# fenghuayumo/DIVSHOT

Hardware: AMD Instinct MI355X
Metric: train views/sec (fwd+bwd raster) at 1M splats 1920x1080 (higher is better)
Workload: dtype f32; 1 GPU; C3: 1000000 splats, 1920x1080, SH degree 3, 8 views per iteration sharded over 1 GPU(s) (BASELINE config C4), 8 view(s) per GPU per step as 1 multi-view pass(es) of 8 view(s) (dvs_raster_forward_views / dvs_raster_backward_*); absgrad=True, mode=batch, stagger=False, groups=1, views_per_group=8, early_gather=False, a9_chunks=1, async_forward=True, hip_graph=False, fwd_variant=quadrant, grad_mode=0, tile_bounds=canonical, shN_layout=tiled[N/64][45][64]

## Files before the change

divshot_amd/csrc/dvs_api.cpp:

```cpp
#include <hip/hip_runtime.h>
#include <cstddef>
#include <cstdio>
#include <cstdlib>
#include <cstdint>
#include <cstring>
#include <mutex>
#include <string>
#include <vector>
#include "../../include/dvs_raster.h"
#include "dvs_kernels.h"

static thread_local std::string g_last_error;
static void set_error(const char* what, hipError_t e, const char* file, int line) {
    char buf[512];
    snprintf(buf, sizeof buf, "%s: %s (%s:%d)", what, hipGetErrorString(e), file, line);
    g_last_error = buf;
}
void dvs_set_last_error(const char* msg) { g_last_error = msg ? msg : ""; }
static int fail(int code, const char* who, const char* what) { g_last_error = std::string(who) + ": " + what; return code; }
#define HIPCHECK(expr) do { hipError_t _e = (expr); if (_e != hipSuccess) { set_error(#expr, _e, __FILE__, __LINE__); return DVS_ERR_HIP; } } while (0)
#define TRY(expr) do { int _r = (expr); if (_r != DVS_OK) return _r; } while (0)

namespace {
struct Buf {
// ... 42 lines not shown

struct FwdPass {
    hipStream_t st;
    const dvs_splats* p; const dvs_camera* cams; int V; const dvs_opts* opts;
    int n; TileGrid g;
    uint64_t T = 0, T_expected = 0;
    const uint64_t* T_dev = nullptr;
    int icur = 0;
    int ranges_encoded = 0;
    bool keys_written = true;
};

struct Arenas {
    Buf radii, splat2d, depth, flags, tiles_touched, rect, rect_sorted, key[2], ids[2];
    Buf ranges, final_T, n_contrib;
    Buf ranges_canon;
    Buf inst_tile[2], inst_splat[2];
    uint64_t inst_cap = 0;
    uint64_t inst_grow_events = 0;
    uint64_t* total_dev = nullptr;
    uint64_t* total_host = nullptr;
    uint64_t overflow_seen = 0;
    Buf tmp_keys, tmp_vals;
};
struct FrontEnd {
    Buf state, hist;
    uint32_t nbv = 0, nsb = 0;
    int rank_atomic = 0;
    DvsSeg *seg_all = nullptr, *seg_vis = nullptr, *seg_tile = nullptr;
    uint32_t *superexcl = nullptr, *totals = nullptr, *block_sums = nullptr, *kred = nullptr, *tile_ranges = nullptr;
// ... 12 lines not shown
    size_t carve_ranges(void* base, int max_views, size_t tiles) {
        Carver k{(char*)base};
        kred = k.take<uint32_t>(DVS_FE_KRED_WORDS);
        super = k.take<unsigned long long>((size_t)max_views * nsb * DVS_FE_SUPER_STRIDE);
        zero_bytes = k.off = (k.off + 255) & ~(size_t)255;
        tile_ranges = k.take<uint32_t>(tiles * 2);
        return k.off;
    }
};
struct Forward {
    dvs_fwd_state st{};
    int n_views = 1;
    bool have = false;
    uint32_t* live_splat = nullptr;
    uint32_t* live_pos = nullptr;
    bool live_lists = true;
    uint64_t* rec_masks = nullptr; uint64_t rec_cap = 0;
    struct Prep {
        bool valid = false;
        int64_t next = 0;
        int n = 0, V = 0;
        dvs_splats p{};
        dvs_opts opts{};
        dvs_camera cams[DVS_MAX_VIEWS];
    } prep;
};
struct Backward {
    Buf g_rows;
    Buf dcolor;
    int variant = DVS_BWD_TR;
    bool keep_rows = false;
// ... 26 lines not shown
    bool async_T = false;
    bool export_tiles = false;
    Arenas a;
    FrontEnd fe;
    Forward fwd;
    Backward bwd;
    Timing timing;
    Probe probe;
    ~dvs_ctx() {
        if (a.total_dev) (void)hipFree(a.total_dev);
        if (a.total_host) (void)hipHostFree(a.total_host);
        for (const auto* pool : {&timing.events, &probe.ev}) for (hipEvent_t e : *pool) (void)hipEventDestroy(e);
    }
};

namespace {
enum : unsigned { DROP_FWD = 1u, DROP_ROWS = 2u, DROP_PREP = 4u, DROP_SEGS = 8u };
void invalidate(dvs_ctx* c, unsigned what) {
    if (what & DROP_FWD) c->fwd.have = false;
    if (what & DROP_ROWS) c->bwd.rows_pending = false;
    if (what & DROP_PREP) c->fwd.prep.valid = false;
    if (what & DROP_SEGS) c->fe.seg_n = -1;
}

struct StageScope {
    dvs_ctx* c; hipStream_t st; bool append; size_t last = 0;
    StageScope(dvs_ctx* c_, hipStream_t s, bool append_) : c(c_), st(s), append(append_) { c->timing.used = 0; c->timing.spans.clear(); }
    size_t mark() {
        Timing& t = c->timing;
        if (!t.on) return 0;
// ... 37 lines not shown
}
int ensure_splat_arenas(dvs_ctx* c, size_t n) {
    Arenas& a = c->a;
    const struct { Buf* buf; size_t each; } need[] = {{&a.radii, 4}, {&a.splat2d, 64}, {&a.depth, 4}, {&a.flags, 4}, {&a.tiles_touched, 4},
        {&a.rect, 16}, {&a.rect_sorted, 16}, {&a.key[0], 4}, {&a.key[1], 4}, {&a.ids[0], 4}, {&a.ids[1], 4}, {&c->bwd.g_rows, 48}};
    for (const auto& x : need) TRY(x.buf->ensure(n * x.each));
    return DVS_OK;
}
int ensure_image_arenas(dvs_ctx* c, int w, int h, int views) {
    const size_t P = (size_t)w * h * views;
    const size_t tiles = (size_t)TileGrid(w, h).tiles * views;
    TRY(c->a.ranges.ensure(c->fe.carve_ranges(nullptr, c->max_views, tiles)));
    c->fe.carve_ranges(c->a.ranges.p, c->max_views, tiles);
    TRY(c->a.ranges_canon.ensure(tiles * 8));
    TRY(c->a.final_T.ensure(P * 4));
    return c->a.n_contrib.ensure(P * 4);
}
int ensure_instance_arenas(dvs_ctx* c, uint64_t T) {
    Arenas& a = c->a;
    if (a.inst_cap && T > a.inst_cap) ++a.inst_grow_events;
    uint64_t cap = (1ull << 32) - 1;
    for (Buf* b : {&a.inst_tile[0], &a.inst_splat[0], &a.inst_tile[1], &a.inst_splat[1]}) {
        TRY(b->ensure(T * 4));
        if (b->bytes / 4 < cap) cap = b->bytes / 4;
    }
    a.inst_cap = cap;
    return c->fe.hist.ensure(dvs_fe_hist_words(a.inst_cap, c->max_views, 512) * 4);
}
}

// ... 151 lines not shown
        HIPCHECK(dvs_launch_seg_sort(st, V, a.inst_tile[0].as<uint32_t>(), a.inst_splat[0].as<uint32_t>(), a.inst_tile[1].as<uint32_t>(),
                                     a.inst_splat[1].as<uint32_t>(), fe.seg_tile, 0, tiles > 1 ? bits_for((uint32_t)(tiles - 1)) : 1,
                                     c->async_T ? (f.T_expected ? f.T_expected : a.inst_cap) : f.T, tile_part, nbtot, fe.hist.as<uint32_t>(), fe.totals,
                                     (uint32_t)tiles, &f.icur, fuse_a6 ? fe.tile_ranges : nullptr, f.keys_written ? 1 : 0, key16, fe.rank_atomic));
    }
    tm.stage("tile_sort");
    if (fuse_a6) f.ranges_encoded = n > 0 ? 1 : 0;
    else HIPCHECK(dvs_launch_tile_ranges(st, f.T, a.inst_tile[f.icur].as<uint32_t>(), fe.tile_ranges, f.T_dev, f.T_expected));
    tm.stage("tile_ranges");
    return DVS_OK;
}
static int fwd_composite_and_publish(dvs_ctx* c, const FwdPass& f, float* out_rgb, dvs_fwd_state* saved, uint64_t* num_rendered, StageScope& tm) {
    Arenas& a = c->a; Forward& fw = c->fwd;
    const int W = f.cams[0].width, H = f.cams[0].height, icur = f.icur;
    probe_event(c, f.st, 0);
    fw.live_splat = nullptr; fw.live_pos = nullptr;
    uint64_t* rec_masks = nullptr; uint64_t rec_cap = 0;
    if (fw.rec_masks && f.V == 1 && !c->async_T) {
        rec_masks = fw.rec_masks; rec_cap = fw.rec_cap;
        HIPCHECK(hipMemsetAsync(rec_masks, 0, (size_t)(f.T < rec_cap ? f.T : rec_cap) * 32, f.st));
    }
    if (fw.live_lists && c->bwd.variant == DVS_BWD_TR) { fw.live_splat = a.inst_splat[icur ^ 1].as<uint32_t>(); fw.live_pos = a.inst_tile[icur ^ 1].as<uint32_t>(); }
    uint32_t* const canon = f.ranges_encoded ? a.ranges_canon.as<uint32_t>() : nullptr;
    HIPCHECK(dvs_launch_render_fwd(f.st, W, H, f.g.tiles_x, f.g.tiles_y, f.V, c->fe.tile_ranges, a.inst_splat[icur].as<uint32_t>(),
                                   a.splat2d.as<float>(), CamVec3(f.cams, f.V, &dvs_camera::bg).v, out_rgb, a.final_T.as<float>(),
                                   a.n_contrib.as<uint32_t>(), fw.live_splat, fw.live_pos, rec_masks, rec_cap, canon));
    probe_event(c, f.st);
    tm.stage("render_fwd");

    dvs_fwd_state& s = fw.st;
    s.radii = a.radii.as<int32_t>(); s.splat2d = a.splat2d.as<float>(); s.depth = a.depth.as<float>();
    s.flags = a.flags.as<uint32_t>();
    s.tiles_touched = a.tiles_touched.as<uint32_t>();
    s.sorted_tile = f.keys_written ? a.inst_tile[icur].as<uint32_t>() : nullptr; s.sorted_splat = a.inst_splat[icur].as<uint32_t>();
    s.ranges = canon ? canon : c->fe.tile_ranges; s.final_T = a.final_T.as<float>(); s.n_contrib = a.n_contrib.as<uint32_t>();
    s.num_rendered = c->async_T ? DVS_T_UNKNOWN : f.T; s.n = f.n; s.width = W; s.height = H; s.tiles_x = f.g.tiles_x; s.tiles_y = f.g.tiles_y;
    s._pad = 0;
    fw.n_views = f.V;
    fw.have = true;
    if (saved) *saved = s;
    if (num_rendered) *num_rendered = s.num_rendered;
// ... 59 lines not shown
    }
    if (count <= 0 || first < 0 || first + count > p->n || (first % 256) != 0) {
        invalidate(c, DROP_PREP);
        return fail(DVS_ERR_INVALID, who, "bad chunk (each starts at a multiple of 256 and lies inside [0, n))");
    }
    HIPCHECK(hipSetDevice(c->device));
    if (begin) invalidate(c, DROP_FWD | DROP_ROWS | DROP_PREP);
    const int r = run_a2(c, (hipStream_t)stream, p, cams, n_views, opts, first, count, begin);
    if (r != DVS_OK) { invalidate(c, DROP_PREP); return r; }
    publish_prep(c, p, cams, n_views, opts, first + count);
    return DVS_OK;
}

int dvs_get_view_state(dvs_ctx* c, int view, dvs_fwd_state* out) {
    if (!c || !out) return fail(DVS_ERR_INVALID, "dvs_get_view_state", "null argument");
    if (!c->fwd.have || view < 0 || view >= c->fwd.n_views) return fail(DVS_ERR_STATE, "dvs_get_view_state", "no such view in the last forward");
    dvs_fwd_state s = c->fwd.st;
    const size_t on = (size_t)view * s.n, op = (size_t)view * s.width * s.height, ot = (size_t)view * s.tiles_x * s.tiles_y;
    s.radii += on; s.splat2d += on * DVS_S2D_FLOATS; s.depth += on; s.flags += on; s.tiles_touched += on;
    s.ranges += 2 * ot; s.final_T += op; s.n_contrib += op;
    *out = s;
    return DVS_OK;
}

static int bwd_composite(dvs_ctx* c, hipStream_t st, const dvs_camera* cams, const dvs_opts* opts, const float* dL_drgb, StageScope& tm) {
    const dvs_fwd_state& s = c->fwd.st;
    Backward& b = c->bwd;
    const int V = c->fwd.n_views;
    tm.begin();
    if (!b.rows_clean) HIPCHECK(hipMemsetAsync(b.g_rows.p, 0, b.g_rows.bytes, st));
    b.rows_clean = false;
    tm.stage("bwd_zero");
    const CamVec3 bgs(cams, V, &dvs_camera::bg);
    probe_event(c, st, 1);
    if (b.variant == DVS_BWD_TR)
        HIPCHECK(dvs_launch_render_bwd_tr(st, s.width, s.height, s.tiles_x, s.tiles_y, V, s.ranges, s.sorted_splat, s.splat2d, bgs.v, s.final_T,
                                          s.n_contrib, dL_drgb, b.g_rows.as<float>(), opts->absgrad, opts->grad_mode, c->fwd.live_splat, c->fwd.live_pos));
    else
        HIPCHECK(dvs_launch_render_bwd_blocks(st, s.width, s.height, s.tiles_x, s.tiles_y, V, s.ranges, s.sorted_splat, s.splat2d,
                                              bgs.v, s.final_T, s.n_contrib, dL_drgb, b.g_rows.as<float>(), opts->absgrad, opts->grad_mode));
    probe_event(c, st);
    tm.stage("render_bwd");
    b.rows_pending = true;
    b.proj_next = 0;
    return DVS_OK;
}
static int bwd_project(dvs_ctx* c, hipStream_t st, const dvs_splats* p, const dvs_camera* cams, const dvs_opts* opts,
                       const dvs_splat_grads* out, int64_t first, int64_t count, StageScope& tm) {
    const dvs_fwd_state& s = c->fwd.st;
    Backward& b = c->bwd;
    const int V = c->fwd.n_views, n = p->n;
    tm.begin();
// ... 251 lines not shown
    c->fwd.rec_masks = take_masks; c->fwd.rec_cap = take_masks ? capacity_instances : 0;
    return DVS_OK;
}

int dvs_set_backward_variant(dvs_ctx* c, int variant) {
    const char* const who = "dvs_set_backward_variant";
    if (!c || variant < DVS_BWD_BLOCKS || variant > DVS_BWD_TR) return fail(DVS_ERR_INVALID, who, "bad argument");
    if (variant == DVS_BWD_REDUCE || variant == DVS_BWD_MM)
        return fail(DVS_ERR_UNSUPPORTED, who, "the 'reduce' and 'mm' kernels are retired — this library contains 'tr' (default) and 'blocks' only");
    c->bwd.variant = variant;
    return DVS_OK;
}
int dvs_set_live_lists(dvs_ctx* c, int enable) {
    if (!c) return fail(DVS_ERR_INVALID, "dvs_set_live_lists", "null context");
    c->fwd.live_lists = enable != 0;
    return DVS_OK;
}
int dvs_set_forward_variant(dvs_ctx* c, int variant) {
    if (!c || (variant != 0 && variant != 1)) return fail(DVS_ERR_INVALID, "dvs_set_forward_variant", "bad argument");
    if (variant == 0)
        return fail(DVS_ERR_UNSUPPORTED, "dvs_set_forward_variant", "the per-block forward is retired — this library contains the quadrant forward only");
    return DVS_OK;
}

int dvs_keep_bwd_intermediates(dvs_ctx* c, int keep) { if (!c) return DVS_ERR_INVALID; c->bwd.keep_rows = keep != 0; return DVS_OK; }

int dvs_get_bwd_intermediates(dvs_ctx* c, const float** rows, int* row_floats) {
    if (!c) return DVS_ERR_INVALID;
    if (rows) *rows = c->bwd.g_rows.as<float>();
    if (row_floats) *row_floats = 12;
// ... 56 lines not shown
```

divshot_amd/csrc/dvs_kernels.h:

```cpp
#pragma once
#include <hip/hip_runtime.h>
#include <stdint.h>
#include "dvs_device.h"

hipError_t dvs_launch_preprocess_fwd(hipStream_t st, int n, const float* pos, const float* sh0, const float* shN,
                                     const float* opacity, const float* scale, const float* rot, const DvsCams& cams, int n_views,
                                     int deg, int antialias, int tiles_x, int tiles_y, int* radii , float* splat2d,
                                     float* depth, uint32_t* flags,
                                     uint32_t* tiles_touched, uint32_t* depth_key, int shn_tiled,
                                     uint32_t* rect , int rect_fmt ,
                                     uint32_t* kred ,
                                     int first, int count );
hipError_t dvs_launch_preprocess_bwd(hipStream_t st, int n, const float* pos, const float* shN, const float* opacity,
                                     const float* scale, const float* rot, const DvsCam& cam, int deg, int antialias,
                                     const int* radii, const uint32_t* flags, float* grad_rows ,
                                     float* g_pos, float* g_sh0, float* g_shN, float* g_opacity, float* g_scale,
                                     float* g_rot, float* out_absgrad2d , float* out_mean2d ,
                                     float* out_dcolor , int accumulate, int rezero_rows, int shn_tiled, int grad_mode);
hipError_t dvs_launch_preprocess_bwd_views(hipStream_t st, int n, int n_views, const float* pos, const float* shN, const float* opacity,
                                           const float* scale, const float* rot, const DvsCams& cams, int deg, int antialias,
                                           const int* radii, const uint32_t* flags, float* grad_rows, float* g_pos, float* g_opacity,
                                           float* g_scale, float* g_rot, float* out_absgrad2d, float* out_mean2d, float* out_dcolor,
                                           int accumulate, int rezero_rows, int grad_mode, int first, int count, float* g_sh0 ,
                                           float* g_shN );
// ... 64 lines not shown
hipError_t dvs_launch_seg_sort(hipStream_t st, int V, uint32_t* keys0, uint32_t* vals0, uint32_t* keys1, uint32_t* vals1, DvsSeg* seg, int bit_lo, int bits,
                               uint64_t grid_elems, uint32_t part, uint32_t nbtot, uint32_t* hist, uint32_t* totals, uint32_t key_add_per_view,
                               int* result_in, uint32_t* ranges_enc = nullptr ,
                               int write_last_keys = 1, int first_keys16 = 0 , int rank_atomic = 0);
hipError_t dvs_fe_probe_rank_atomic(hipStream_t st, uint32_t* bad_dev);
hipError_t dvs_launch_seg_binning(hipStream_t st, int n, int V, int rect_fmt, const DvsSeg* seg_vis, DvsSeg* seg_tile, const uint32_t* sorted_ids,
                                  const uint32_t* rect, uint32_t* rect_sorted, uint32_t* block_sums, unsigned long long* super, uint32_t* superexcl,
                                  uint32_t tile_part, unsigned long long* total_dev, unsigned long long capacity, int stage, int tiles_x,
                                  uint32_t* inst_tile, uint32_t* inst_splat, int key16 = 0 );

hipError_t dvs_launch_tile_ranges(hipStream_t st, uint64_t T, const uint32_t* sorted_tile, uint32_t* ranges ,
                                  const uint64_t* T_dev = nullptr, uint64_t T_expected = 0);
hipError_t dvs_launch_export_keys(hipStream_t st, uint64_t T, const uint32_t* sorted_tile, const uint32_t* sorted_splat,
                                  const float* depth, uint64_t* out_keys);

hipError_t dvs_launch_render_fwd(hipStream_t st, int W, int H, int tiles_x, int tiles_y, int n_views, const uint32_t* ranges ,
                                 const uint32_t* sorted_splat, const float* splat2d, const float* bgs, float* out_color, float* final_T,
                                 uint32_t* n_contrib, uint32_t* live_splat , uint32_t* live_pos ,
                                 uint64_t* take_masks ,
                                 uint64_t take_cap, uint32_t* ranges_out = nullptr );
enum { DVS_BWD_BLOCKS = 0 , DVS_BWD_REDUCE = 1 , DVS_BWD_MM = 2 ,
       DVS_BWD_TR = 3  };

hipError_t dvs_launch_render_bwd_tr(hipStream_t st, int W, int H, int tiles_x, int tiles_y, int n_views, const uint32_t* ranges,
                                    const uint32_t* sorted_splat, const float* splat2d, const float* bgs , const float* final_T,
                                    const uint32_t* n_contrib, const float* dL_dout, float* grad_rows, int absgrad, int grad_mode,
                                    const uint32_t* live_splat ,
                                    const uint32_t* live_pos);

hipError_t dvs_launch_render_bwd_blocks(hipStream_t st, int W, int H, int tiles_x, int tiles_y, int n_views, const uint32_t* ranges,
                                        const uint32_t* sorted_splat, const float* splat2d, const float* bgs , const float* final_T,
                                        const uint32_t* n_contrib, const float* dL_dout, float* grad_rows, int absgrad, int grad_mode);
```

divshot_amd/csrc/render.hip:

```cpp
#include "dvs_device.h"
#include "dvs_kernels.h"
#include "render_common.h"

struct __attribute__((aligned(16))) FwdLds {
    float4 a[RB];
    float4 b[RB];
    float4 c[RB];
    uint64_t qmask[RB / 64][4];
    uint32_t wlive[RB / 64];
};
__device__ __forceinline__ void lds_put(FwdLds& L, int t, float2 xy, float4 co, float3 col) {
    L.a[t] = make_float4(xy.x, xy.y, -0.72134752044448170f * co.x, -1.4426950408889634f * co.y);
    L.b[t] = make_float4(-0.72134752044448170f * co.z, co.w, col.x, col.y);
    L.c[t].x = col.z;
}

__device__ __forceinline__ bool stage_batch(FwdLds& L, const uint32_t* __restrict__ sorted_splat, uint32_t first, int cnt,
                                            const float4* __restrict__ splat2d, float tile_x0, float tile_y0, uint32_t& id_out) {
    const int t = threadIdx.x;
    uint32_t qm = 0;
    id_out = 0u;
    if (t < cnt) {
        const uint32_t id = sorted_splat[first + t];
        id_out = id;
// ... 37 lines not shown
}

__device__ __forceinline__ uint64_t uniform_u64(uint64_t v) {
    const uint32_t lo = __builtin_amdgcn_readfirstlane((uint32_t)v), hi = __builtin_amdgcn_readfirstlane((uint32_t)(v >> 32));
    return ((uint64_t)hi << 32) | lo;
}

template <bool RECORD>
__global__ void __launch_bounds__(RB)
k_render_fwd(ViewBg bg_arg , int W, int H, int tiles_x, int tiles_per_view,
             int num_tiles , const uint2* __restrict__ ranges, uint2* __restrict__ ranges_out ,
             const uint32_t* __restrict__ sorted_splat, const float4* __restrict__ splat2d,
             float* __restrict__ out_color , float* __restrict__ final_T , uint32_t* __restrict__ n_contrib,
             uint32_t* __restrict__ live_splat ,
             uint32_t* __restrict__ live_pos ,
             uint64_t* __restrict__ take_masks , uint64_t take_cap) {
    __shared__ FwdLds L;
    (void)bg_arg;
    const int tile_g = tile_of_block(blockIdx.x, num_tiles);
    if (tile_g >= num_tiles) return;
    const int view = tile_g / tiles_per_view, tile = tile_g - view * tiles_per_view;
    const float3 bgv = dvs_load_bg(view);
    const float bg0 = bgv.x, bg1 = bgv.y, bg2 = bgv.z;
    out_color += (size_t)view * 3 * W * H; final_T += (size_t)view * W * H; n_contrib += (size_t)view * W * H;
    const int tx = tile % tiles_x, ty = tile / tiles_x;
    const int wave = threadIdx.x >> 6, lane = threadIdx.x & 63;
    const int px = tx * DVS_TILE + (wave & 1) * 8 + (lane & 7);
    const int py = ty * DVS_TILE + (wave >> 1) * 8 + (lane >> 3);
    const bool inside = px < W && py < H;
    const float pxf = (float)px, pyf = (float)py;
    uint2 range = ranges[tile_g];
    if (ranges_out) {
        range.x = range.y ? ~range.x : 0u;
        if (threadIdx.x == 0) ranges_out[tile_g] = range;
    }
    const int total = (int)(range.y - range.x);
    uint64_t notdone = __builtin_amdgcn_ballot_w64(inside);
    float T = 1.0f, C0 = 0.f, C1 = 0.f, C2 = 0.f;
    uint32_t last = 0;
    uint32_t live_base = 0;

    for (int base = 0; base < total; base += RB) {
        if (__syncthreads_and(notdone == 0ull)) break;
        const int cnt = min(RB, total - base);
        uint32_t my_id;
        const bool live = stage_batch(L, sorted_splat, range.x + base, cnt, splat2d, (float)(tx * DVS_TILE), (float)(ty * DVS_TILE), my_id);
        const uint64_t lm = __ballot(live);
        const uint32_t lrank = __builtin_amdgcn_mbcnt_hi((uint32_t)(lm >> 32), __builtin_amdgcn_mbcnt_lo((uint32_t)lm, 0u));
        if (lane == 0) L.wlive[wave] = (uint32_t)__popcll(lm);
        __syncthreads();
        if (live_pos) {
            uint32_t pre = 0, tot = 0;
#pragma unroll
            for (int w = 0; w < RB / 64; ++w) { const uint32_t c = L.wlive[w]; pre += w < wave ? c : 0u; tot += c; }
            const uint32_t lp = live_base + pre + lrank;
            if ((int)threadIdx.x < cnt) live_pos[range.x + base + threadIdx.x] = lp;
            if (live) live_splat[range.x + lp] = my_id;
            live_base += tot;
        }
        if (notdone == 0ull) continue;
#pragma unroll 1
        for (int lw = 0; lw < RB / 64; ++lw) {
            uint64_t m = uniform_u64(L.qmask[lw][wave]);
            if (m == 0) continue;
            if (notdone == 0ull) break;
            typedef float fwd_v4f __attribute__((ext_vector_type(4)));
            typedef __attribute__((address_space(3))) const fwd_v4f lds_cv4f;
            uint32_t word_a = (uint32_t)(uintptr_t)&L.a[lw * 64];
            asm("" : "+v"(word_a));
            const int idx0 = base + lw * 64 + 1;
            uint64_t exec_entry;
            asm volatile("s_mov_b64 %0, exec" : "=s"(exec_entry));
// ... 25 lines not shown
                             "v_mov_b32 %[last], %[idx]\n\t"
                             "s_mov_b64 exec, %[ee]"
                             : [c0] "+v"(C0), [c1] "+v"(C1), [c2] "+v"(C2), [T] "+v"(T), [last] "+v"(last), [nd] "+s"(notdone)
                             : [p2] "v"(p2), [al] "v"(alpha), [tt] "v"(test_T), [cr] "v"(B.z), [cg] "v"(B.w), [cbl] "v"(cb), [at] "v"(aT), [idx] "s"(idx),
                               [amin] "s"(DVS_ALPHA_MIN), [tstop] "s"(DVS_T_STOP), [ee] "s"(exec_entry)
                             : "vcc", "scc");
                if (RECORD) {
                    const uint64_t took = nd_before & __builtin_amdgcn_ballot_w64(!(p2 > 0.f)) & __builtin_amdgcn_ballot_w64(!(alpha < DVS_ALPHA_MIN)) &
                                          ~__builtin_amdgcn_ballot_w64(test_T < DVS_T_STOP);
                    const uint64_t pos = (uint64_t)range.x + (uint64_t)(idx - 1u);
                    if (lane == 0 && pos < take_cap) take_masks[pos * 4 + wave] = took;
                }
            }
        }
    }
    if (inside) {
        const size_t P = (size_t)W * H, pix = (size_t)py * W + px;
        final_T[pix] = T;
        n_contrib[pix] = last;
        out_color[pix] = C0 + T * bg0;
        out_color[P + pix] = C1 + T * bg1;
        out_color[2 * P + pix] = C2 + T * bg2;
    }
}


hipError_t dvs_launch_render_fwd(hipStream_t st, int W, int H, int tiles_x, int tiles_y, int n_views, const uint32_t* ranges,
                                 const uint32_t* sorted_splat, const float* splat2d, const float* bgs, float* out_color, float* final_T,
                                 uint32_t* n_contrib, uint32_t* live_splat, uint32_t* live_pos, uint64_t* take_masks, uint64_t take_cap, uint32_t* ranges_out) {
    const int tiles_pv = tiles_x * tiles_y, num_tiles = tiles_pv * n_views;
    if (num_tiles <= 0) return hipSuccess;
    const int grid = ((num_tiles + 7) >> 3) << 3;
    if (take_masks)
        hipLaunchKernelGGL(k_render_fwd<true>, dim3(grid), dim3(RB), 0, st, make_view_bg(n_views, bgs), W, H, tiles_x, tiles_pv, num_tiles,
                           (const uint2*)ranges, (uint2*)ranges_out, sorted_splat, (const float4*)splat2d, out_color, final_T, n_contrib, live_splat, live_pos, take_masks, take_cap);
    else
        hipLaunchKernelGGL(k_render_fwd<false>, dim3(grid), dim3(RB), 0, st, make_view_bg(n_views, bgs), W, H, tiles_x, tiles_pv, num_tiles,
                           (const uint2*)ranges, (uint2*)ranges_out, sorted_splat, (const float4*)splat2d, out_color, final_T, n_contrib, live_splat, live_pos, (uint64_t*)nullptr, (uint64_t)0);
    return hipGetLastError();
}
```

divshot_amd/csrc/render_tr.hip:

```cpp
#include "dvs_device.h"
#include "dvs_kernels.h"
#include "render_common.h"

#define TR_SLOTS 4
#define TR_SS 136
#define TR_MINW 6

template <int BK>
struct __attribute__((aligned(16))) TrLds {
    float4 ea[BK + 1];
    float4 eb[BK + 1];
    float4 ec[BK + 1];
    uint2 idop[2][BK];
    uint8_t list[(BK + 1) * 16];
    uint32_t cnt[16];
    uint32_t blast[16];
};

template <int BK>
__device__ __forceinline__ uint32_t tr_load_id(const uint32_t* __restrict__ sorted_splat, uint32_t first, int cnt) {
    const int e = threadIdx.x % BK;
    return e < cnt ? sorted_splat[first + e] : 0u;
}
template <int BK>
// ... 48 lines not shown
            len = (uint32_t)__popc(up ? hi : lo);
        }
        if (hit) L.list[(rk + 1u) * 16u + (uint32_t)(b0 + i)] = (uint8_t)e;
        if (e == 0) L.cnt[b0 + i] = len;
    }
}

template <bool ABSGRAD, bool LINEAGE, int BK>
__global__ void __launch_bounds__(RB, TR_MINW)
k_render_bwd_tr(ViewBg bg_arg , int W, int H, int tiles_x, int tiles_per_view,
                int num_tiles , const uint2* __restrict__ ranges,
                const uint32_t* __restrict__ sorted_splat, const float4* __restrict__ splat2d,
                const float* __restrict__ final_T, const uint32_t* __restrict__ n_contrib, const float* __restrict__ dL_dout ,
                float* __restrict__ grow ,
                const uint32_t* __restrict__ live_splat ,
                const uint32_t* __restrict__ live_pos ) {
    __shared__ TrLds<BK> L;
    __shared__ __attribute__((aligned(16))) float s_tab[4][(BK + 1) * 12];
    __shared__ __attribute__((aligned(16))) float s_tb[4][TR_SLOTS * TR_SS];
    (void)bg_arg;
    const int tile_g = tile_of_block(blockIdx.x, num_tiles);
    if (tile_g >= num_tiles) return;
    const int view = tile_g / tiles_per_view, tile = tile_g - view * tiles_per_view;
    const float3 bgv = dvs_load_bg(view);
    final_T += (size_t)view * W * H; n_contrib += (size_t)view * W * H; dL_dout += (size_t)view * 3 * W * H;
    const int tx = tile % tiles_x, ty = tile / tiles_x;
    const int wave = threadIdx.x >> 6, lane = threadIdx.x & 63;
    const size_t P = (size_t)W * H;
    const int g1 = lane >> 4, pi = lane & 15;
    const int bx1 = 2 * (wave & 1) + (g1 & 1), by1 = 2 * (wave >> 1) + (g1 >> 1), blk1 = by1 * 4 + bx1;
    const int px = tx * DVS_TILE + 4 * bx1 + (pi & 3), py = ty * DVS_TILE + 4 * by1 + (pi >> 2);
    const bool inside = px < W && py < H;
    const size_t pix = (size_t)py * W + px;
    const float pxf = (float)px, pyf = (float)py;
    const uint2 range = ranges[tile_g];
    const int r2 = lane >> 4, s2 = (lane >> 2) & 3, g2 = lane & 3;
    const int bx2 = 2 * (wave & 1) + (g2 & 1), by2 = 2 * (wave >> 1) + (g2 >> 1);
    const int X0 = tx * DVS_TILE + 4 * bx2, Y0 = ty * DVS_TILE + 4 * by2 + r2;
    const float X0f = (float)X0, Y0f = (float)Y0;
    float d2[4][3];
    if ((W & 3) == 0) {
        const bool in2 = X0 < W && Y0 < H;
        const size_t q = (size_t)Y0 * W + X0;
#pragma unroll
        for (int c = 0; c < 3; ++c) {
            const float4 v = in2 ? *reinterpret_cast<const float4*>(dL_dout + c * P + q) : make_float4(0.f, 0.f, 0.f, 0.f);
            d2[0][c] = v.x; d2[1][c] = v.y; d2[2][c] = v.z; d2[3][c] = v.w;
        }
    } else {
#pragma unroll
        for (int x = 0; x < 4; ++x) {
            const bool in2 = X0 + x < W && Y0 < H;
            const size_t q = (size_t)Y0 * W + X0 + x;
#pragma unroll
            for (int c = 0; c < 3; ++c) d2[x][c] = in2 ? dL_dout[c * P + q] : 0.f;
        }
    }
    const int perm_r = (r2 == 1) ? 2 : (r2 == 2) ? 1 : r2;
    const int xaddr = (lane ^ 32) << 2;
    const int jaddr = (16 * g2) << 2;
    const uint32_t jshift = 8u * (uint32_t)(TR_SLOTS - 1 - s2);

    const float T_final = inside ? final_T[pix] : 0.f;
    uint32_t last = inside ? n_contrib[pix] : 0u;
    if (live_pos) {
        if (last > 0u) last = live_pos[range.x + last - 1u] + 1u;
        sorted_splat = live_splat;
    }
    float dLp0 = 0.f, dLp1 = 0.f, dLp2 = 0.f;
    if (inside) { dLp0 = dL_dout[pix]; dLp1 = dL_dout[P + pix]; dLp2 = dL_dout[2 * P + pix]; }
    const float bg_dot = (bgv.x * dLp0 + bgv.y * dLp1) + bgv.z * dLp2;

    uint32_t bmax = last;
#pragma unroll
    for (int d = 8; d >= 1; d >>= 1) bmax = max(bmax, (uint32_t)__shfl_xor((int)bmax, d, 64));
    if (pi == 0) L.blast[blk1] = bmax;
    for (int e = threadIdx.x; e < (BK + 1) * 12; e += RB) reinterpret_cast<float4*>(&s_tab[0][0])[e] = make_float4(0.f, 0.f, 0.f, 0.f);
    if (threadIdx.x < 16) L.list[threadIdx.x] = (uint8_t)BK;
    if (threadIdx.x == 0) { L.ea[BK] = make_float4(0.f, 0.f, 0.f, 0.f); L.eb[BK] = make_float4(0.f, 0.f, 0.f, 0.f); L.ec[BK] = make_float4(0.f, 0.f, 0.f, 0.f); }
    __syncthreads();
    uint32_t todo = 0;
#pragma unroll
    for (int g = 0; g < 16; ++g) todo = max(todo, L.blast[g]);
    if (todo == 0) return;

    float T = T_final;
    float D = T_final * bg_dot;
    const uint32_t tb_m0 = (uint32_t)__builtin_amdgcn_readfirstlane((int)(uint32_t)(uintptr_t)&s_tb[wave][0]);
    typedef __attribute__((address_space(3))) float lds_float;
    typedef float tr_v4f __attribute__((ext_vector_type(4)));
    typedef __attribute__((address_space(3))) const tr_v4f lds_cv4f;
    uint32_t tbr_a = (uint32_t)(uintptr_t)&s_tb[wave][TR_SS * s2 + 16 * g2 + 4 * r2];
    uint32_t tabw_a = (uint32_t)(uintptr_t)&s_tab[wave][perm_r];
    asm("" : "+v"(tbr_a), "+v"(tabw_a));
    const uint8_t* const lbase = &L.list[0];

    auto flush = [&](uint32_t jpack) {
        const uint32_t jp = (uint32_t)__builtin_amdgcn_ds_bpermute(jaddr, (int)jpack);
        const int j = (int)((jp >> jshift) & 0xffu);
// ... 36 lines not shown
        }
        const float q0 = swap16_add(h0, h1), q1 = swap16_add(h2, h3), q2 = swap16_add(h4, h5);
        uint32_t slot_a;
        asm("v_mad_u32_u24 %0, %1, 48, %2" : "=v"(slot_a) : "v"(j), "v"(tabw_a));
        lds_float* const slot = (lds_float*)slot_a;
#pragma unroll
        for (int g = 0; g < 4; ++g) {
            if (g2 == g) { slot[0] += q0; slot[4] += q1; slot[8] += q2; }
            __builtin_amdgcn_wave_barrier();
            asm volatile("" ::: "memory");
        }
    };

    const int nbatch = (int)((todo + BK - 1) / BK);
    const float tile_x0 = (float)(tx * DVS_TILE), tile_y0 = (float)(ty * DVS_TILE);
    uint32_t id_stage = tr_load_id<BK>(sorted_splat, range.x + (nbatch - 1) * BK, min(BK, (int)todo - (nbatch - 1) * BK));
    for (int b = nbatch - 1; b >= 0; --b) {
        const int base = b * BK;
        const int cnt = min(BK, (int)todo - base);
        tr_stage<BK>(L, splat2d, id_stage, cnt, base, b & 1, tile_x0, tile_y0);
        __syncthreads();
        const int len = (int)L.cnt[blk1];
        int nmax = len;
        nmax = max(nmax, __shfl_xor(nmax, 16, 64));
        nmax = max(nmax, __shfl_xor(nmax, 32, 64));
        nmax = __builtin_amdgcn_readfirstlane(nmax);
        const int lastb = (int)min(last, (uint32_t)(base + BK)) - base;
        uint32_t p = (uint32_t)len * 16u + (uint32_t)blk1;
        uint32_t jn = lbase[p];
        asm("" : "+v"(jn));
        uint32_t jpack = 0;
// ... 43 lines not shown
            const float val = (s_tab[0][e] + s_tab[1][e]) + (s_tab[2][e] + s_tab[3][e]);
            if (val != 0.f) {
                const int ent = e / 12, comp = e - 12 * ent;
                const uint2 io = L.idop[b & 1][ent];
                const float sc = (comp == 5 || (comp >= 6 && comp <= 8)) ? 1.f : __uint_as_float(io.y);
                if (comp < 11) atomicAdd(&grow[(size_t)io.x * 12 + comp], val * sc);
            }
            s_tab[0][e] = 0.f; s_tab[1][e] = 0.f; s_tab[2][e] = 0.f; s_tab[3][e] = 0.f;
        }
    }
}

hipError_t dvs_launch_render_bwd_tr(hipStream_t st, int W, int H, int tiles_x, int tiles_y, int n_views, const uint32_t* ranges,
                                    const uint32_t* sorted_splat, const float* splat2d, const float* bgs, const float* final_T,
                                    const uint32_t* n_contrib, const float* dL_dout, float* grad_rows, int absgrad, int grad_mode,
                                    const uint32_t* live_splat, const uint32_t* live_pos) {
    const int tiles_pv = tiles_x * tiles_y, num_tiles = tiles_pv * n_views;
    if (num_tiles <= 0) return hipSuccess;
    const int grid = ((num_tiles + 7) >> 3) << 3;
    const int lineage = grad_mode == 1 ? 1 : 0;
#define DVS_TR(A, LN, BKV)                                                                                                              \
    hipLaunchKernelGGL((k_render_bwd_tr<A, LN, BKV>), dim3(grid), dim3(RB), 0, st, make_view_bg(n_views, bgs), W, H, tiles_x, tiles_pv, \
                       num_tiles, (const uint2*)ranges, sorted_splat, (const float4*)splat2d, final_T, n_contrib, dL_dout, grad_rows, live_splat, live_pos)
#define DVS_TR_B(BKV)                                                                                   \
    do {                                                                                                \
        if (absgrad) { if (lineage) DVS_TR(true, true, BKV); else DVS_TR(true, false, BKV); }           \
        else { if (lineage) DVS_TR(false, true, BKV); else DVS_TR(false, false, BKV); }                 \
    } while (0)
    DVS_TR_B(64);
#undef DVS_TR_B
#undef DVS_TR
    return hipGetLastError();
}
```

include/dvs_raster.h:

```cpp
#ifndef DVS_RASTER_H
#define DVS_RASTER_H

#include <stddef.h>
#include <stdint.h>

#ifdef __cplusplus
extern "C" {
#endif

#define DVS_TILE 16
#define DVS_SH_REST 15

enum {
    DVS_OK = 0,
    DVS_ERR_INVALID = 1,
    DVS_ERR_HIP = 2,
    DVS_ERR_CAPACITY = 3,
    DVS_ERR_STATE = 4,
    DVS_ERR_UNSUPPORTED = 5
};

typedef struct dvs_splats {
    const float* pos;
    const float* sh0;
// ... 87 lines not shown

int dvs_sh_grad_combine(dvs_ctx* ctx, void* stream, int n, const float* pos, int sh_degree, int n_views, const float* campos,
                        const float* dcolor, float* g_sh0, float* g_shN, int accumulate, int shn_layout);
int dvs_shn_relayout(dvs_ctx* ctx, void* stream, int n, const float* src, float* dst, int to_tiled);

dvs_ctx* dvs_create_views(int device, size_t max_splats, int max_w, int max_h, int max_views);
int dvs_raster_forward_views(dvs_ctx* ctx, void* stream, const dvs_splats* params, const dvs_camera* cams, int n_views,
                             const dvs_opts* opts, float* out_rgb);
int dvs_raster_backward_views(dvs_ctx* ctx, void* stream, const dvs_splats* params, const dvs_camera* cams, int n_views,
                              const dvs_opts* opts, const float* dL_drgb, const dvs_splat_grads* out);

int dvs_raster_forward_views_prepare(dvs_ctx* ctx, void* stream, const dvs_splats* params, const dvs_camera* cams, int n_views,
                                     const dvs_opts* opts, int64_t first, int64_t count);
int dvs_raster_forward_cancel_prepared(dvs_ctx* ctx);
int dvs_get_view_state(dvs_ctx* ctx, int view, dvs_fwd_state* state);

#define DVS_T_UNKNOWN (~0ull)
int dvs_set_async(dvs_ctx* ctx, int enable);
int dvs_get_num_rendered(dvs_ctx* ctx, void* stream, uint64_t* num_rendered);
int dvs_get_arena_info(dvs_ctx* ctx, uint64_t* instance_capacity, uint64_t* grow_events, uint64_t* last_num_rendered, uint64_t* overflows);
int dvs_get_sort_rank_mode(dvs_ctx* ctx);
int dvs_set_export_sorted_tiles(dvs_ctx* ctx, int enable);

int dvs_debug_record_decisions(dvs_ctx* ctx, uint64_t* take_masks, uint64_t capacity_instances);
int dvs_debug_sort_depth_keys(dvs_ctx* ctx, void* stream, const uint32_t* keys, uint64_t n, uint32_t* sorted_ids, uint32_t* n_sorted, uint32_t* digit_bits);

int dvs_set_backward_variant(dvs_ctx* ctx, int variant);
int dvs_set_forward_variant(dvs_ctx* ctx, int variant);
int dvs_set_live_lists(dvs_ctx* ctx, int enable);

// ... 24 lines not shown
```

Measured before the change: 1830 views/s.

## Hand off per-pixel live count and per-tile block maxima from forward to backward

The forward render kernel now also writes a compacted per-pixel last-live index and a per-tile header holding the tile's todo count and its 16 block maxima. The backward TR kernel reads these instead of gathering live_pos through n_contrib and reducing block maxima with shuffles and LDS, and it issues the first id stage load earlier. This removes a dependent indirect load and a reduction plus sync from the backward prologue. In exchange the forward kernel gains extra LDS, shuffles, a barrier and additional global writes of a pixel-sized buffer.

```diff
diff --git a/divshot_amd/csrc/dvs_api.cpp b/divshot_amd/csrc/dvs_api.cpp
--- a/divshot_amd/csrc/dvs_api.cpp
+++ b/divshot_amd/csrc/dvs_api.cpp
@@ -80,6 +80,7 @@
 struct Arenas {
     Buf radii, splat2d, depth, flags, tiles_touched, rect, rect_sorted, key[2], ids[2];
     Buf ranges, final_T, n_contrib;
+    Buf last_live, tile_head;
     Buf ranges_canon;
     Buf inst_tile[2], inst_splat[2];
     uint64_t inst_cap = 0;
@@ -122,7 +123,10 @@
     bool have = false;
     uint32_t* live_splat = nullptr;
     uint32_t* live_pos = nullptr;
+    uint32_t* last_live = nullptr;
+    DvsTileHead* tile_head = nullptr;
     bool live_lists = true;
+    bool use_handoff = true;
     uint64_t* rec_masks = nullptr; uint64_t rec_cap = 0;
     struct Prep {
         bool valid = false;
@@ -179,6 +183,7 @@
     }
 };
 
+static_assert(sizeof(DvsTileHead) == 4 * DVS_TILE_HEAD_WORDS, "dvs_raster.h describes the tile header to the tests");
 namespace {
 enum : unsigned { DROP_FWD = 1u, DROP_ROWS = 2u, DROP_PREP = 4u, DROP_SEGS = 8u };
 void invalidate(dvs_ctx* c, unsigned what) {
@@ -246,6 +251,8 @@
     c->fe.carve_ranges(c->a.ranges.p, c->max_views, tiles);
     TRY(c->a.ranges_canon.ensure(tiles * 8));
     TRY(c->a.final_T.ensure(P * 4));
+    TRY(c->a.last_live.ensure(P * 4));
+    TRY(c->a.tile_head.ensure(tiles * sizeof(DvsTileHead)));
     return c->a.n_contrib.ensure(P * 4);
 }
 int ensure_instance_arenas(dvs_ctx* c, uint64_t T) {
@@ -427,17 +434,18 @@
     Arenas& a = c->a; Forward& fw = c->fwd;
     const int W = f.cams[0].width, H = f.cams[0].height, icur = f.icur;
     probe_event(c, f.st, 0);
-    fw.live_splat = nullptr; fw.live_pos = nullptr;
+    fw.live_splat = nullptr; fw.live_pos = nullptr; fw.last_live = nullptr; fw.tile_head = nullptr;
     uint64_t* rec_masks = nullptr; uint64_t rec_cap = 0;
     if (fw.rec_masks && f.V == 1 && !c->async_T) {
         rec_masks = fw.rec_masks; rec_cap = fw.rec_cap;
         HIPCHECK(hipMemsetAsync(rec_masks, 0, (size_t)(f.T < rec_cap ? f.T : rec_cap) * 32, f.st));
     }
     if (fw.live_lists && c->bwd.variant == DVS_BWD_TR) { fw.live_splat = a.inst_splat[icur ^ 1].as<uint32_t>(); fw.live_pos = a.inst_tile[icur ^ 1].as<uint32_t>(); }
+    if (fw.live_pos && !rec_masks) { fw.last_live = a.last_live.as<uint32_t>(); fw.tile_head = a.tile_head.as<DvsTileHead>(); }
     uint32_t* const canon = f.ranges_encoded ? a.ranges_canon.as<uint32_t>() : nullptr;
     HIPCHECK(dvs_launch_render_fwd(f.st, W, H, f.g.tiles_x, f.g.tiles_y, f.V, c->fe.tile_ranges, a.inst_splat[icur].as<uint32_t>(),
                                    a.splat2d.as<float>(), CamVec3(f.cams, f.V, &dvs_camera::bg).v, out_rgb, a.final_T.as<float>(),
-                                   a.n_contrib.as<uint32_t>(), fw.live_splat, fw.live_pos, rec_masks, rec_cap, canon));
+                                   a.n_contrib.as<uint32_t>(), fw.live_splat, fw.live_pos, rec_masks, rec_cap, canon, fw.last_live, fw.tile_head));
     probe_event(c, f.st);
     tm.stage("render_fwd");
 
@@ -527,6 +535,13 @@
 
 int dvs_get_view_state(dvs_ctx* c, int view, dvs_fwd_state* out) {
     if (!c || !out) return fail(DVS_ERR_INVALID, "dvs_get_view_state", "null argument");
+    if (c->fwd.have && view == DVS_VIEW_HANDOFF) {
+        dvs_fwd_state s = c->fwd.st;
+        s.sorted_splat = c->fwd.live_splat; s.sorted_tile = c->fwd.live_pos; s.n_contrib = c->fwd.last_live;
+        s.tiles_touched = reinterpret_cast<const uint32_t*>(c->fwd.tile_head);
+        *out = s;
+        return DVS_OK;
+    }
     if (!c->fwd.have || view < 0 || view >= c->fwd.n_views) return fail(DVS_ERR_STATE, "dvs_get_view_state", "no such view in the last forward");
     dvs_fwd_state s = c->fwd.st;
     const size_t on = (size_t)view * s.n, op = (size_t)view * s.width * s.height, ot = (size_t)view * s.tiles_x * s.tiles_y;
@@ -548,7 +563,8 @@
     probe_event(c, st, 1);
     if (b.variant == DVS_BWD_TR)
         HIPCHECK(dvs_launch_render_bwd_tr(st, s.width, s.height, s.tiles_x, s.tiles_y, V, s.ranges, s.sorted_splat, s.splat2d, bgs.v, s.final_T,
-                                          s.n_contrib, dL_drgb, b.g_rows.as<float>(), opts->absgrad, opts->grad_mode, c->fwd.live_splat, c->fwd.live_pos));
+                                          s.n_contrib, dL_drgb, b.g_rows.as<float>(), opts->absgrad, opts->grad_mode, c->fwd.live_splat, c->fwd.live_pos,
+                                          c->fwd.use_handoff ? c->fwd.last_live : nullptr, c->fwd.use_handoff ? c->fwd.tile_head : nullptr));
     else
         HIPCHECK(dvs_launch_render_bwd_blocks(st, s.width, s.height, s.tiles_x, s.tiles_y, V, s.ranges, s.sorted_splat, s.splat2d,
                                               bgs.v, s.final_T, s.n_contrib, dL_drgb, b.g_rows.as<float>(), opts->absgrad, opts->grad_mode));
@@ -830,6 +846,7 @@
 int dvs_set_live_lists(dvs_ctx* c, int enable) {
     if (!c) return fail(DVS_ERR_INVALID, "dvs_set_live_lists", "null context");
     c->fwd.live_lists = enable != 0;
+    c->fwd.use_handoff = enable != 2;
     return DVS_OK;
 }
 int dvs_set_forward_variant(dvs_ctx* c, int variant) {
diff --git a/divshot_amd/csrc/dvs_kernels.h b/divshot_amd/csrc/dvs_kernels.h
--- a/divshot_amd/csrc/dvs_kernels.h
+++ b/divshot_amd/csrc/dvs_kernels.h
@@ -102,11 +102,20 @@
 hipError_t dvs_launch_export_keys(hipStream_t st, uint64_t T, const uint32_t* sorted_tile, const uint32_t* sorted_splat,
                                   const float* depth, uint64_t* out_keys);
 
+struct __attribute__((aligned(16))) DvsTileHead {
+    uint32_t todo;
+    uint32_t blast[16];
+    uint32_t _pad[3];
+};
+static_assert(sizeof(DvsTileHead) == 80, "DvsTileHead: 20 words (DVS_TILE_HEAD_WORDS of dvs_raster.h)");
+
 hipError_t dvs_launch_render_fwd(hipStream_t st, int W, int H, int tiles_x, int tiles_y, int n_views, const uint32_t* ranges ,
                                  const uint32_t* sorted_splat, const float* splat2d, const float* bgs, float* out_color, float* final_T,
                                  uint32_t* n_contrib, uint32_t* live_splat , uint32_t* live_pos ,
                                  uint64_t* take_masks ,
-                                 uint64_t take_cap, uint32_t* ranges_out = nullptr );
+                                 uint64_t take_cap, uint32_t* ranges_out = nullptr ,
+                                 uint32_t* last_live = nullptr ,
+                                 DvsTileHead* tile_head = nullptr );
 enum { DVS_BWD_BLOCKS = 0 , DVS_BWD_REDUCE = 1 , DVS_BWD_MM = 2 ,
        DVS_BWD_TR = 3  };
 
@@ -114,7 +123,9 @@
                                     const uint32_t* sorted_splat, const float* splat2d, const float* bgs , const float* final_T,
                                     const uint32_t* n_contrib, const float* dL_dout, float* grad_rows, int absgrad, int grad_mode,
                                     const uint32_t* live_splat ,
-                                    const uint32_t* live_pos);
+                                    const uint32_t* live_pos,
+                                    const uint32_t* last_live = nullptr ,
+                                    const DvsTileHead* tile_head = nullptr );
 
 hipError_t dvs_launch_render_bwd_blocks(hipStream_t st, int W, int H, int tiles_x, int tiles_y, int n_views, const uint32_t* ranges,
                                         const uint32_t* sorted_splat, const float* splat2d, const float* bgs , const float* final_T,
diff --git a/divshot_amd/csrc/render.hip b/divshot_amd/csrc/render.hip
--- a/divshot_amd/csrc/render.hip
+++ b/divshot_amd/csrc/render.hip
@@ -8,6 +8,7 @@
     float4 c[RB];
     uint64_t qmask[RB / 64][4];
     uint32_t wlive[RB / 64];
+    uint32_t lp[RB];
 };
 __device__ __forceinline__ void lds_put(FwdLds& L, int t, float2 xy, float4 co, float3 col) {
     L.a[t] = make_float4(xy.x, xy.y, -0.72134752044448170f * co.x, -1.4426950408889634f * co.y);
@@ -75,7 +76,9 @@
              float* __restrict__ out_color , float* __restrict__ final_T , uint32_t* __restrict__ n_contrib,
              uint32_t* __restrict__ live_splat ,
              uint32_t* __restrict__ live_pos ,
-             uint64_t* __restrict__ take_masks , uint64_t take_cap) {
+             uint64_t* __restrict__ take_masks , uint64_t take_cap,
+             uint32_t* __restrict__ last_live ,
+             DvsTileHead* __restrict__ tile_head ) {
     __shared__ FwdLds L;
     (void)bg_arg;
     const int tile_g = tile_of_block(blockIdx.x, num_tiles);
@@ -100,9 +103,14 @@
     float T = 1.0f, C0 = 0.f, C1 = 0.f, C2 = 0.f;
     uint32_t last = 0;
     uint32_t live_base = 0;
-
-    for (int base = 0; base < total; base += RB) {
-        if (__syncthreads_and(notdone == 0ull)) break;
+    const bool handoff = live_pos != nullptr && tile_head != nullptr;
+    uint32_t ll = 0;
+
+    int base = 0;
+    for (; base < total; base += RB) {
+        const bool all_done = __syncthreads_and(notdone == 0ull);
+        if (handoff && (int)last > base - RB && base > 0) ll = L.lp[(int)last - 1 - (base - RB)] + 1u;
+        if (all_done) break;
         const int cnt = min(RB, total - base);
         uint32_t my_id;
         const bool live = stage_batch(L, sorted_splat, range.x + base, cnt, splat2d, (float)(tx * DVS_TILE), (float)(ty * DVS_TILE), my_id);
@@ -117,6 +125,7 @@
             const uint32_t lp = live_base + pre + lrank;
             if ((int)threadIdx.x < cnt) live_pos[range.x + base + threadIdx.x] = lp;
             if (live) live_splat[range.x + lp] = my_id;
+            if (handoff) L.lp[threadIdx.x] = lp;
             live_base += tot;
         }
         if (notdone == 0ull) continue;
@@ -172,8 +181,25 @@
             }
         }
     }
+    if (handoff) {
+        if (base >= total && total > 0) {
+            __syncthreads();
+            if ((int)last > base - RB) ll = L.lp[(int)last - 1 - (base - RB)] + 1u;
+        }
+        uint32_t bm = ll;
+        bm = max(bm, (uint32_t)__shfl_xor((int)bm, 1, 64)); bm = max(bm, (uint32_t)__shfl_xor((int)bm, 2, 64));
+        bm = max(bm, (uint32_t)__shfl_xor((int)bm, 8, 64)); bm = max(bm, (uint32_t)__shfl_xor((int)bm, 16, 64));
+        uint32_t wm = max(bm, (uint32_t)__shfl_xor((int)bm, 4, 64));
+        wm = max(wm, (uint32_t)__shfl_xor((int)wm, 32, 64));
+        DvsTileHead* const th = tile_head + tile_g;
+        if ((lane & 0x1b) == 0) th->blast[(2 * (wave >> 1) + (lane >> 5)) * 4 + 2 * (wave & 1) + ((lane >> 2) & 1)] = bm;
+        if (lane == 0) L.wlive[wave] = wm;
+        __syncthreads();
+        if (threadIdx.x == 0) th->todo = max(max(L.wlive[0], L.wlive[1]), max(L.wlive[2], L.wlive[3]));
+    }
     if (inside) {
         const size_t P = (size_t)W * H, pix = (size_t)py * W + px;
+        if (handoff) last_live[(size_t)view * P + pix] = ll;
         final_T[pix] = T;
         n_contrib[pix] = last;
         out_color[pix] = C0 + T * bg0;
@@ -185,15 +211,17 @@
 
 hipError_t dvs_launch_render_fwd(hipStream_t st, int W, int H, int tiles_x, int tiles_y, int n_views, const uint32_t* ranges,
                                  const uint32_t* sorted_splat, const float* splat2d, const float* bgs, float* out_color, float* final_T,
-                                 uint32_t* n_contrib, uint32_t* live_splat, uint32_t* live_pos, uint64_t* take_masks, uint64_t take_cap, uint32_t* ranges_out) {
+                                 uint32_t* n_contrib, uint32_t* live_splat, uint32_t* live_pos, uint64_t* take_masks, uint64_t take_cap, uint32_t* ranges_out,
+                                 uint32_t* last_live, DvsTileHead* tile_head) {
     const int tiles_pv = tiles_x * tiles_y, num_tiles = tiles_pv * n_views;
     if (num_tiles <= 0) return hipSuccess;
     const int grid = ((num_tiles + 7) >> 3) << 3;
+    if (!live_pos || !last_live || !tile_head) { last_live = nullptr; tile_head = nullptr; }
     if (take_masks)
         hipLaunchKernelGGL(k_render_fwd<true>, dim3(grid), dim3(RB), 0, st, make_view_bg(n_views, bgs), W, H, tiles_x, tiles_pv, num_tiles,
-                           (const uint2*)ranges, (uint2*)ranges_out, sorted_splat, (const float4*)splat2d, out_color, final_T, n_contrib, live_splat, live_pos, take_masks, take_cap);
+                           (const uint2*)ranges, (uint2*)ranges_out, sorted_splat, (const float4*)splat2d, out_color, final_T, n_contrib, live_splat, live_pos, take_masks, take_cap, last_live, tile_head);
     else
         hipLaunchKernelGGL(k_render_fwd<false>, dim3(grid), dim3(RB), 0, st, make_view_bg(n_views, bgs), W, H, tiles_x, tiles_pv, num_tiles,
-                           (const uint2*)ranges, (uint2*)ranges_out, sorted_splat, (const float4*)splat2d, out_color, final_T, n_contrib, live_splat, live_pos, (uint64_t*)nullptr, (uint64_t)0);
+                           (const uint2*)ranges, (uint2*)ranges_out, sorted_splat, (const float4*)splat2d, out_color, final_T, n_contrib, live_splat, live_pos, (uint64_t*)nullptr, (uint64_t)0, last_live, tile_head);
     return hipGetLastError();
 }
diff --git a/divshot_amd/csrc/render_tr.hip b/divshot_amd/csrc/render_tr.hip
--- a/divshot_amd/csrc/render_tr.hip
+++ b/divshot_amd/csrc/render_tr.hip
@@ -86,7 +86,9 @@
                 const float* __restrict__ final_T, const uint32_t* __restrict__ n_contrib, const float* __restrict__ dL_dout ,
                 float* __restrict__ grow ,
                 const uint32_t* __restrict__ live_splat ,
-                const uint32_t* __restrict__ live_pos ) {
+                const uint32_t* __restrict__ live_pos ,
+                const uint32_t* __restrict__ last_live ,
+                const DvsTileHead* __restrict__ tile_head ) {
     __shared__ TrLds<BK> L;
     __shared__ __attribute__((aligned(16))) float s_tab[4][(BK + 1) * 12];
     __shared__ __attribute__((aligned(16))) float s_tb[4][TR_SLOTS * TR_SS];
@@ -106,6 +108,9 @@
     const size_t pix = (size_t)py * W + px;
     const float pxf = (float)px, pyf = (float)py;
     const uint2 range = ranges[tile_g];
+    const bool handoff = live_pos != nullptr && tile_head != nullptr;
+    if (live_pos) sorted_splat = live_splat;
+    uint32_t todo = handoff ? tile_head[tile_g].todo : 0u, id_stage = 0;
     const int r2 = lane >> 4, s2 = (lane >> 2) & 3, g2 = lane & 3;
     const int bx2 = 2 * (wave & 1) + (g2 & 1), by2 = 2 * (wave >> 1) + (g2 >> 1);
     const int X0 = tx * DVS_TILE + 4 * bx2, Y0 = ty * DVS_TILE + 4 * by2 + r2;
@@ -128,33 +133,44 @@
             for (int c = 0; c < 3; ++c) d2[x][c] = in2 ? dL_dout[c * P + q] : 0.f;
         }
     }
+    if (handoff) {
+        if (todo == 0) return;
+        const int nb = (int)((todo + BK - 1) / BK);
+        id_stage = tr_load_id<BK>(sorted_splat, range.x + (nb - 1) * BK, min(BK, (int)todo - (nb - 1) * BK));
+    }
     const int perm_r = (r2 == 1) ? 2 : (r2 == 2) ? 1 : r2;
     const int xaddr = (lane ^ 32) << 2;
     const int jaddr = (16 * g2) << 2;
     const uint32_t jshift = 8u * (uint32_t)(TR_SLOTS - 1 - s2);
 
     const float T_final = inside ? final_T[pix] : 0.f;
-    uint32_t last = inside ? n_contrib[pix] : 0u;
-    if (live_pos) {
-        if (last > 0u) last = live_pos[range.x + last - 1u] + 1u;
-        sorted_splat = live_splat;
+    uint32_t last;
+    if (handoff) last = inside ? last_live[(size_t)view * P + pix] : 0u;
+    else {
+        last = inside ? n_contrib[pix] : 0u;
+        if (live_pos && last > 0u) last = live_pos[range.x + last - 1u] + 1u;
     }
     float dLp0 = 0.f, dLp1 = 0.f, dLp2 = 0.f;
     if (inside) { dLp0 = dL_dout[pix]; dLp1 = dL_dout[P + pix]; dLp2 = dL_dout[2 * P + pix]; }
     const float bg_dot = (bgv.x * dLp0 + bgv.y * dLp1) + bgv.z * dLp2;
 
-    uint32_t bmax = last;
-#pragma unroll
-    for (int d = 8; d >= 1; d >>= 1) bmax = max(bmax, (uint32_t)__shfl_xor((int)bmax, d, 64));
-    if (pi == 0) L.blast[blk1] = bmax;
+    if (handoff) {
+        if (threadIdx.x < 16) L.blast[threadIdx.x] = tile_head[tile_g].blast[threadIdx.x];
+    } else {
+        uint32_t bmax = last;
+#pragma unroll
+        for (int d = 8; d >= 1; d >>= 1) bmax = max(bmax, (uint32_t)__shfl_xor((int)bmax, d, 64));
+        if (pi == 0) L.blast[blk1] = bmax;
+    }
     for (int e = threadIdx.x; e < (BK + 1) * 12; e += RB) reinterpret_cast<float4*>(&s_tab[0][0])[e] = make_float4(0.f, 0.f, 0.f, 0.f);
     if (threadIdx.x < 16) L.list[threadIdx.x] = (uint8_t)BK;
     if (threadIdx.x == 0) { L.ea[BK] = make_float4(0.f, 0.f, 0.f, 0.f); L.eb[BK] = make_float4(0.f, 0.f, 0.f, 0.f); L.ec[BK] = make_float4(0.f, 0.f, 0.f, 0.f); }
     __syncthreads();
-    uint32_t todo = 0;
-#pragma unroll
-    for (int g = 0; g < 16; ++g) todo = max(todo, L.blast[g]);
-    if (todo == 0) return;
+    if (!handoff) {
+#pragma unroll
+        for (int g = 0; g < 16; ++g) todo = max(todo, L.blast[g]);
+        if (todo == 0) return;
+    }
 
     float T = T_final;
     float D = T_final * bg_dot;
@@ -221,7 +237,7 @@
 
     const int nbatch = (int)((todo + BK - 1) / BK);
     const float tile_x0 = (float)(tx * DVS_TILE), tile_y0 = (float)(ty * DVS_TILE);
-    uint32_t id_stage = tr_load_id<BK>(sorted_splat, range.x + (nbatch - 1) * BK, min(BK, (int)todo - (nbatch - 1) * BK));
+    if (!handoff) id_stage = tr_load_id<BK>(sorted_splat, range.x + (nbatch - 1) * BK, min(BK, (int)todo - (nbatch - 1) * BK));
     for (int b = nbatch - 1; b >= 0; --b) {
         const int base = b * BK;
         const int cnt = min(BK, (int)todo - base);
@@ -295,14 +311,15 @@
 hipError_t dvs_launch_render_bwd_tr(hipStream_t st, int W, int H, int tiles_x, int tiles_y, int n_views, const uint32_t* ranges,
                                     const uint32_t* sorted_splat, const float* splat2d, const float* bgs, const float* final_T,
                                     const uint32_t* n_contrib, const float* dL_dout, float* grad_rows, int absgrad, int grad_mode,
-                                    const uint32_t* live_splat, const uint32_t* live_pos) {
+                                    const uint32_t* live_splat, const uint32_t* live_pos, const uint32_t* last_live, const DvsTileHead* tile_head) {
     const int tiles_pv = tiles_x * tiles_y, num_tiles = tiles_pv * n_views;
     if (num_tiles <= 0) return hipSuccess;
     const int grid = ((num_tiles + 7) >> 3) << 3;
+    if (!live_pos || !last_live || !tile_head) { last_live = nullptr; tile_head = nullptr; }
     const int lineage = grad_mode == 1 ? 1 : 0;
 #define DVS_TR(A, LN, BKV)                                                                                                              \
     hipLaunchKernelGGL((k_render_bwd_tr<A, LN, BKV>), dim3(grid), dim3(RB), 0, st, make_view_bg(n_views, bgs), W, H, tiles_x, tiles_pv, \
-                       num_tiles, (const uint2*)ranges, sorted_splat, (const float4*)splat2d, final_T, n_contrib, dL_dout, grad_rows, live_splat, live_pos)
+                       num_tiles, (const uint2*)ranges, sorted_splat, (const float4*)splat2d, final_T, n_contrib, dL_dout, grad_rows, live_splat, live_pos, last_live, tile_head)
 #define DVS_TR_B(BKV)                                                                                   \
     do {                                                                                                \
         if (absgrad) { if (lineage) DVS_TR(true, true, BKV); else DVS_TR(true, false, BKV); }           \
diff --git a/include/dvs_raster.h b/include/dvs_raster.h
--- a/include/dvs_raster.h
+++ b/include/dvs_raster.h
@@ -125,6 +125,8 @@
                                      const dvs_opts* opts, int64_t first, int64_t count);
 int dvs_raster_forward_cancel_prepared(dvs_ctx* ctx);
 int dvs_get_view_state(dvs_ctx* ctx, int view, dvs_fwd_state* state);
+#define DVS_VIEW_HANDOFF (-1)
+#define DVS_TILE_HEAD_WORDS 20
 
 #define DVS_T_UNKNOWN (~0ull)
 int dvs_set_async(dvs_ctx* ctx, int enable);
```

Result: no change. 1827 views/s (-0.2%).
